# RenYurui/Global-Flow-Local-Attention

Hardware: AMD Instinct MI355X
Metric: images/sec (fwd+bwd) PoseGenerator 256x176 attn_layer=2,3 -- feature-warping hot path (higher is better)
Workload: dtype f32 (FC products: 2-term f16 splits exact to 2^-24 on f16 MFMA, f32 accumulate)

## Files before the change

### global_flow_local_attention_amd/csrc/fc_conv_impl.h

```cpp
#pragma once

#include "fc_mma.h"

namespace gfla {

constexpr int kFcMinRowBlocks = 2, kFcMaxRowBlocks = 8;
constexpr int kFcPrefetch = 8;

template <int MODE>
__device__ __forceinline__ void load_b_frags(Frag<MODE> (&fb)[Fc<MODE>::KB], const unsigned char *p, int64_t split_stride) {
  if constexpr (MODE == 0) {
    fb[0].v = *reinterpret_cast<const float4 *>(p);
    fb[1].v = *reinterpret_cast<const float4 *>(p + 32);
  } else {
#pragma unroll
    for (int sp = 0; sp < Fc<MODE>::NS; ++sp) fb[0].s[sp] = *reinterpret_cast<const f16x8 *>(p + sp * split_stride);
  }
}

typedef unsigned int u32x4 __attribute__((ext_vector_type(4)));

__device__ __forceinline__ void fc_prefetch_pieces(u32x4 (&pf)[kFcPrefetch], const unsigned char *src, int x_ps, int pix0,
                                                   int tmh) {
#pragma unroll
  for (int q = 0; q < kFcPrefetch; ++q)
    pf[q] = *reinterpret_cast<const u32x4 *>(src + (int64_t)min(pix0 + 64 * q, tmh - 1) * x_ps);
}

struct ConvTiling {
  int T, base, rem, heavy, per_ntile;
};

template <int MODE, int KS, int NMB, bool SRC32 = false>
__global__ __launch_bounds__(256, 2) void fc_conv_kernel(PackedDesc X, const unsigned char *__restrict__ Wk,
                                                        int64_t w_split_stride, float *__restrict__ out,
                                                        int64_t out_bs, int ldo, int n_valid, int M, int Wv, int Wp,
                                                        int nch, int tmh, ConvTiling tl,
                                                        const uint32_t *__restrict__ amax_x,
                                                        const uint32_t *__restrict__ amax_w) {
  using F = Fc<MODE>;
  constexpr int KK = KS * KS, PITCH = F::PITCH, STEPS = F::KB * NMB;
  extern __shared__ __attribute__((aligned(16))) unsigned char gfla_smem[];
  unsigned char *xs = gfla_smem;
  const int t = threadIdx.x, lane = t & 63, wave = t >> 6, l31 = lane & 31, kh = lane >> 5;
  int wid = blockIdx.x;
  const int ntile = wid / tl.per_ntile;
  wid -= ntile * tl.per_ntile;
  if (tl.per_ntile <= 2 * kNumCU && wid >= kNumCU) wid = tl.per_ntile - 1 - (wid - kNumCU);
  else if (tl.per_ntile <= kNumCU && (ntile & 1)) wid = tl.per_ntile - 1 - wid;
  int64_t b;
  int first, nblk;
  if (wid < tl.heavy) {
    b = wid / tl.rem;
    first = (wid - (int)b * tl.rem) * (tl.base + 1);
    nblk = tl.base + 1;
  } else {
    const int u = wid - tl.heavy, per = tl.T - tl.rem;
    b = u / per;
    first = tl.rem * (tl.base + 1) + (u - (int)b * per) * tl.base;
    nblk = tl.base;
  }
  const int m0 = first * 32;
  const int y0 = m0 / Wv, p0 = y0 * Wp + (m0 - y0 * Wv);
  const int64_t x_ss = X.split_stride, x_cs = X.chunk_stride;
  const int x_ps = X.pix_stride;
  const unsigned char *xg = X.base + b * X.batch_stride + (int64_t)p0 * x_ps;
  constexpr int64_t kWTile = (int64_t)kFcTN * F::REC;
  const unsigned char *wg = Wk + (int64_t)ntile * nch * KK * kWTile + (wave * 32 + l31) * F::REC + kh * 16;

  int a_off[NMB];
#pragma unroll
  for (int mb = 0; mb < NMB; ++mb) {
    const int r = min(m0 + mb * 32 + l31, M - 1);
    const int y = r / Wv;
    a_off[mb] = (y * Wp + (r - y * Wv) - p0) * PITCH;
  }

  f32x16 acc[NMB];
#pragma unroll
  for (int mb = 0; mb < NMB; ++mb)
#pragma unroll
    for (int r = 0; r < 16; ++r) acc[mb][r] = 0.f;

  static_assert(!SRC32 || MODE == 2, "float32 source: mode 2 arithmetic only");
  const int per = tmh * (SRC32 ? 4 : F::PIECES);
  const int x_total = SRC32 ? per : per * F::NS;
  const int xplane = tmh * PITCH;

  constexpr int PF = kFcPrefetch;
  constexpr bool kPrefetch = MODE == 0 || SRC32;
  const float sx32 = SRC32 ? fc_scale(amax_x) : 1.f;
  auto store_split = [&](unsigned char *dst8, u32x4 v) {
    uint32_t h01, l01, h23, l23;
    fc_split_pair(__uint_as_float(v[0]) * sx32, __uint_as_float(v[1]) * sx32, h01, l01);
    fc_split_pair(__uint_as_float(v[2]) * sx32, __uint_as_float(v[3]) * sx32, h23, l23);
    *reinterpret_cast<uint2 *>(dst8) = make_uint2(h01, h23);
    *reinterpret_cast<uint2 *>(dst8 + xplane) = make_uint2(l01, l23);
  };
  u32x4 pf[PF];
  const int pix0 = t >> 2;
  const unsigned char *pf_src = xg + (t & 3) * 16;
  unsigned char *pf_dst = xs + (size_t)pix0 * PITCH + (t & 3) * (SRC32 ? 8 : 16);
  const int x_first = kPrefetch ? min(x_total, 256 * PF) : 0;

  Frag<MODE> cur[F::KB], nxt[F::KB];
  load_b_frags<MODE>(cur, wg, w_split_stride);
  if constexpr (kPrefetch) fc_prefetch_pieces(pf, pf_src, x_ps, pix0, tmh);
  for (int cc = 0; cc < nch; ++cc) {
    __syncthreads();
    if constexpr (kPrefetch) {
#pragma unroll
      for (int q = 0; q < PF; ++q)
        if (pix0 + 64 * q < tmh) {
          if constexpr (SRC32) store_split(pf_dst + (size_t)q * 64 * PITCH, pf[q]);
          else *reinterpret_cast<u32x4 *>(pf_dst + (size_t)q * 64 * PITCH) = pf[q];
        }
    }
    if constexpr (SRC32) {
      const unsigned char *src = xg + (int64_t)cc * x_cs + (t & 3) * 16;
      for (int pix = pix0 + 64 * PF; pix < tmh; pix += 64)
        store_split(xs + (size_t)pix * PITCH + (t & 3) * 8, *reinterpret_cast<const u32x4 *>(src + (int64_t)pix * x_ps));
    } else if (x_first < x_total) {
      const unsigned char *src = xg + (int64_t)cc * x_cs;
      for (int base = x_first + t; base < x_total; base += 256 * 4) {
        uint4 v0 = make_uint4(0, 0, 0, 0), v1 = v0, v2 = v0, v3 = v0;
#define GFLA_X_SP(idx_) (((idx_) >= per) + ((idx_) >= 2 * per))
#define GFLA_X_REM(idx_) ((idx_)-GFLA_X_SP(idx_) * per)
#define GFLA_X_SRC(idx_) \
  (src + GFLA_X_SP(idx_) * x_ss + (int64_t)(GFLA_X_REM(idx_) / F::PIECES) * x_ps + (GFLA_X_REM(idx_) % F::PIECES) * 16)
#define GFLA_X_DST(idx_) \
  (xs + ((size_t)GFLA_X_SP(idx_) * tmh + GFLA_X_REM(idx_) / F::PIECES) * PITCH + (GFLA_X_REM(idx_) % F::PIECES) * 16)
        if (base < x_total) v0 = *reinterpret_cast<const uint4 *>(GFLA_X_SRC(base));
        if (base + 256 < x_total) v1 = *reinterpret_cast<const uint4 *>(GFLA_X_SRC(base + 256));
        if (base + 512 < x_total) v2 = *reinterpret_cast<const uint4 *>(GFLA_X_SRC(base + 512));
        if (base + 768 < x_total) v3 = *reinterpret_cast<const uint4 *>(GFLA_X_SRC(base + 768));
        if (base < x_total) *reinterpret_cast<uint4 *>(GFLA_X_DST(base)) = v0;
        if (base + 256 < x_total) *reinterpret_cast<uint4 *>(GFLA_X_DST(base + 256)) = v1;
        if (base + 512 < x_total) *reinterpret_cast<uint4 *>(GFLA_X_DST(base + 512)) = v2;
        if (base + 768 < x_total) *reinterpret_cast<uint4 *>(GFLA_X_DST(base + 768)) = v3;
#undef GFLA_X_SRC
#undef GFLA_X_DST
#undef GFLA_X_SP
#undef GFLA_X_REM
      }
    }
    __syncthreads();
    Frag<MODE> fa = load_frag<MODE>(xs + a_off[0], xplane, 0, kh);
#pragma unroll 1
    for (int tap = 0; tap < KK; ++tap) {
      {
        const int lin = cc * KK + tap + 1;
#pragma unroll
        for (int q = 0; q < F::KB; ++q) nxt[q] = cur[q];
        if (lin < nch * KK) load_b_frags<MODE>(nxt, wg + (int64_t)lin * kWTile, w_split_stride);
        if constexpr (kPrefetch)
          if (tap == 0 && cc + 1 < nch)
            fc_prefetch_pieces(pf, pf_src + (int64_t)(cc + 1) * x_cs, x_ps, pix0, tmh);
      }
      const int i = tap / KS, j = tap - i * KS;
      const unsigned char *xa = xs + (size_t)(i * Wp + j) * PITCH;
      const int tn = tap + 1 < KK ? tap + 1 : 0;
      const int in = tn / KS, jn = tn - in * KS;
      const unsigned char *xa_next = xs + (size_t)(in * Wp + jn) * PITCH;
#pragma unroll
      for (int st = 0; st < STEPS; ++st) {
        const int kb = st / NMB, mb = st % NMB;
        const Frag<MODE> fc = fa;
        if (st + 1 < STEPS)
          fa = load_frag<MODE>(xa + a_off[(st + 1) % NMB], xplane, (st + 1) / NMB, kh);
        else
          fa = load_frag<MODE>(xa_next + a_off[0], xplane, 0, kh);
        __builtin_amdgcn_sched_barrier(0);
        if (mb + 1 < NMB || nblk == NMB)
          acc[mb] = mma<MODE>(fc, cur[kb], acc[mb]);
      }
#pragma unroll
      for (int q = 0; q < F::KB; ++q) cur[q] = nxt[q];
    }
  }

  const float inv = MODE == 0 ? 1.f : fc_inv_scale(amax_x) * fc_inv_scale(amax_w);
  float *ob = out + b * out_bs;
  const int col = ntile * kFcTN + wave * 32 + l31;
  if (col < n_valid) {
#pragma unroll
    for (int mb = 0; mb < NMB; ++mb) {
      if (mb >= nblk) continue;
#pragma unroll
      for (int r = 0; r < 16; ++r) {
        const int m = m0 + mb * 32 + (r & 3) + 8 * (r >> 2) + 4 * kh;
        if (m < M) ob[(int64_t)m * ldo + col] = acc[mb][r] * inv;
      }
    }
  }
}



inline int fc_conv_tile_pixels(int mb, int Wv, int Wp, int k) {
  const int tm = 32 * mb;
  return tm + ((tm - 1) / Wv + 1) * (Wp - Wv) + (k - 1) * (Wp + 1);
}

inline int pick_conv_tiling(int M, int64_t B, int ntiles_n, int Wv, int Wp, int k, int mode, ConvTiling *tl) {
  const int ns = fc_nsplit(mode), pitch = mode ? 48 : 80;
  const int nb = (int)ceil_div(M, 32);
  const int forced = tuning(11);
  int64_t T = (2 * kNumCU) / (B * ntiles_n);
  if (T < 1) T = 1;
  if (T > nb) T = nb;
  if (ceil_div(nb, T) > kFcMaxRowBlocks) T = ceil_div(nb, kFcMaxRowBlocks);
  if (forced >= kFcMinRowBlocks && forced <= kFcMaxRowBlocks) T = ceil_div(nb, forced);
  for (;; ++T) {
    const int nmb = (int)ceil_div(nb, T);
    const int64_t lds = (int64_t)ns * fc_conv_tile_pixels(nmb < kFcMinRowBlocks ? kFcMinRowBlocks : nmb, Wv, Wp, k) * pitch;
    if (lds <= 156 * 1024) break;
    if (nmb <= kFcMinRowBlocks) return 0;
  }
  tl->T = (int)T;
  tl->base = nb / (int)T;
  tl->rem = nb % (int)T;
  tl->heavy = (int)B * tl->rem;
  tl->per_ntile = (int)(B * T);
  int nmb = tl->base + (tl->rem ? 1 : 0);
  if (nmb < kFcMinRowBlocks) {
    nmb = kFcMinRowBlocks;
  }
  return nmb;
}

template <int MODE, int KS, int NMB, bool SRC32 = false>
static int launch_conv(const PackedDesc &X, const void *wk, int64_t w_split_stride, float *out, int64_t out_bs,
                       int ldo, int n_valid, int64_t B, int nch, int M, int Wv, int Wp, const ConvTiling &tl,
                       const uint32_t *amax_x, const uint32_t *amax_w, hipStream_t stream) {
  using F = Fc<MODE>;
  const int tmh = fc_conv_tile_pixels(NMB, Wv, Wp, KS);
  const unsigned lds = (unsigned)(F::NS * tmh * F::PITCH);
  const int64_t wgs = (int64_t)tl.per_ntile * ceil_div(n_valid, kFcTN);
  if (wgs > 0x7fffffffLL) return GFLA_ERR_UNSUPPORTED;
  auto kern = fc_conv_kernel<MODE, KS, NMB, SRC32>;
  if (lds > 64 * 1024)
    (void)hipFuncSetAttribute(reinterpret_cast<const void *>(kern), hipFuncAttributeMaxDynamicSharedMemorySize, (int)lds);
  kern<<<dim3((unsigned)wgs), 256, lds, stream>>>(X, static_cast<const unsigned char *>(wk), w_split_stride, out, out_bs,
                                                  ldo, n_valid, M, Wv, Wp, nch, tmh, tl, amax_x, amax_w);
  return launch_status();
}

template <int MODE, int KS, bool SRC32 = false>
static int dispatch_conv(int nmb, const PackedDesc &X, const void *wk, int64_t wss, float *out, int64_t out_bs, int ldo,
                         int n_valid, int64_t B, int nch, int M, int Wv, int Wp, const ConvTiling &tl, const uint32_t *ax,
                         const uint32_t *aw, hipStream_t s) {
  switch (nmb) {
#define GFLA_CASE(N_) \
  case N_: return launch_conv<MODE, KS, N_, SRC32>(X, wk, wss, out, out_bs, ldo, n_valid, B, nch, M, Wv, Wp, tl, ax, aw, s)
    GFLA_CASE(2);
    GFLA_CASE(3);
    GFLA_CASE(4);
    GFLA_CASE(5);
    GFLA_CASE(6);
    GFLA_CASE(7);
    GFLA_CASE(8);
#undef GFLA_CASE
  }
  return GFLA_ERR_UNSUPPORTED;
}

template <int MODE>
int fc_conv_mode(const PackedDesc &X, const void *wk, int64_t w_split_stride, float *out, int64_t out_bs, int ldo,
                 int n_valid, int64_t B, int nch, int M, int Wv, int Wp, int k, const uint32_t *amax_x,
                 const uint32_t *amax_w, hipStream_t stream);

#define GFLA_DEFINE_FC_CONV_MODE(MODE_)                                                                               \
  template <>                                                                                                         \
  int fc_conv_mode<MODE_>(const PackedDesc &X, const void *wk, int64_t w_split_stride, float *out, int64_t out_bs,    \
                          int ldo, int n_valid, int64_t B, int nch, int M, int Wv, int Wp, int k,                     \
                          const uint32_t *amax_x, const uint32_t *amax_w, hipStream_t stream) {                       \
    ConvTiling tl;                                                                                                    \
    const int nmb = pick_conv_tiling(M, B, (int)ceil_div(n_valid, kFcTN), Wv, Wp, k, MODE_, &tl);                      \
    if (nmb == 0) return GFLA_ERR_UNSUPPORTED;                                                                        \
    if (k == 3)                                                                                                       \
      return dispatch_conv<MODE_, 3>(nmb, X, wk, w_split_stride, out, out_bs, ldo, n_valid, B, nch, M, Wv, Wp, tl,     \
                                     amax_x, amax_w, stream);                                                         \
    return dispatch_conv<MODE_, 5>(nmb, X, wk, w_split_stride, out, out_bs, ldo, n_valid, B, nch, M, Wv, Wp, tl,       \
                                   amax_x, amax_w, stream);                                                           \
  }

}
```

Measured before the change: 9591.

## Ring-buffer weight fragments two taps ahead and load via buffer resources

```diff
diff --git a/global_flow_local_attention_amd/csrc/fc_conv_impl.h b/global_flow_local_attention_amd/csrc/fc_conv_impl.h
--- a/global_flow_local_attention_amd/csrc/fc_conv_impl.h
+++ b/global_flow_local_attention_amd/csrc/fc_conv_impl.h
@@ -6,25 +6,33 @@
 
 constexpr int kFcMinRowBlocks = 2, kFcMaxRowBlocks = 8;
 constexpr int kFcPrefetch = 8;
+constexpr int kFcWeightAhead = 2, kFcRingMaxRowBlocks = 7;
+
+typedef unsigned int u32x4 __attribute__((ext_vector_type(4)));
+
+__device__ __forceinline__ __amdgpu_buffer_rsrc_t fc_rsrc(const unsigned char *base) {
+  return __builtin_amdgcn_make_buffer_rsrc(const_cast<unsigned char *>(base), 0, -1, 0x00020000);
+}
 
 template <int MODE>
-__device__ __forceinline__ void load_b_frags(Frag<MODE> (&fb)[Fc<MODE>::KB], const unsigned char *p, int64_t split_stride) {
+__device__ __forceinline__ void load_b_frags(Frag<MODE> (&fb)[Fc<MODE>::KB], const __amdgpu_buffer_rsrc_t (&w)[Fc<MODE>::NS],
+                                             int tile_off, int lane_off) {
   if constexpr (MODE == 0) {
-    fb[0].v = *reinterpret_cast<const float4 *>(p);
-    fb[1].v = *reinterpret_cast<const float4 *>(p + 32);
+    fb[0].v = __builtin_bit_cast(float4, __builtin_amdgcn_raw_buffer_load_b128(w[0], lane_off, tile_off, 0));
+    fb[1].v = __builtin_bit_cast(float4, __builtin_amdgcn_raw_buffer_load_b128(w[0], lane_off + 32, tile_off, 0));
   } else {
 #pragma unroll
-    for (int sp = 0; sp < Fc<MODE>::NS; ++sp) fb[0].s[sp] = *reinterpret_cast<const f16x8 *>(p + sp * split_stride);
-  }
-}
-
-typedef unsigned int u32x4 __attribute__((ext_vector_type(4)));
-
-__device__ __forceinline__ void fc_prefetch_pieces(u32x4 (&pf)[kFcPrefetch], const unsigned char *src, int x_ps, int pix0,
-                                                   int tmh) {
+    for (int sp = 0; sp < Fc<MODE>::NS; ++sp)
+      fb[0].s[sp] = __builtin_bit_cast(f16x8, __builtin_amdgcn_raw_buffer_load_b128(w[sp], lane_off, tile_off, 0));
+  }
+}
+
+__device__ __forceinline__ void fc_prefetch_pieces(u32x4 (&pf)[kFcPrefetch], const unsigned char *tile, int x_ps, int pix0,
+                                                   int tmh, int piece_off) {
+  const __amdgpu_buffer_rsrc_t x = fc_rsrc(tile);
 #pragma unroll
   for (int q = 0; q < kFcPrefetch; ++q)
-    pf[q] = *reinterpret_cast<const u32x4 *>(src + (int64_t)min(pix0 + 64 * q, tmh - 1) * x_ps);
+    pf[q] = __builtin_amdgcn_raw_buffer_load_b128(x, min(pix0 + 64 * q, tmh - 1) * x_ps + piece_off, 0, 0);
 }
 
 struct ConvTiling {
@@ -66,7 +74,10 @@
   const int x_ps = X.pix_stride;
   const unsigned char *xg = X.base + b * X.batch_stride + (int64_t)p0 * x_ps;
   constexpr int64_t kWTile = (int64_t)kFcTN * F::REC;
-  const unsigned char *wg = Wk + (int64_t)ntile * nch * KK * kWTile + (wave * 32 + l31) * F::REC + kh * 16;
+  const int w_lane = (wave * 32 + l31) * F::REC + kh * 16;
+  __amdgpu_buffer_rsrc_t wg[F::NS];
+#pragma unroll
+  for (int sp = 0; sp < F::NS; ++sp) wg[sp] = fc_rsrc(Wk + (int64_t)ntile * nch * KK * kWTile + sp * w_split_stride);
 
   int a_off[NMB];
 #pragma unroll
@@ -99,13 +110,18 @@
   };
   u32x4 pf[PF];
   const int pix0 = t >> 2;
-  const unsigned char *pf_src = xg + (t & 3) * 16;
+  const int pf_piece = (t & 3) * 16;
   unsigned char *pf_dst = xs + (size_t)pix0 * PITCH + (t & 3) * (SRC32 ? 8 : 16);
   const int x_first = kPrefetch ? min(x_total, 256 * PF) : 0;
 
-  Frag<MODE> cur[F::KB], nxt[F::KB];
-  load_b_frags<MODE>(cur, wg, w_split_stride);
-  if constexpr (kPrefetch) fc_prefetch_pieces(pf, pf_src, x_ps, pix0, tmh);
+  constexpr int TU = KS == 3 && NMB <= kFcRingMaxRowBlocks ? KK : 1, AHEAD = TU == 1 ? 1 : kFcWeightAhead;
+  static_assert(KK % TU == 0 && AHEAD >= 1 && (TU == 1 || AHEAD < TU), "ring: a slot per tap phase, reused after it has been read");
+  const int lin_last = nch * KK - 1;
+  Frag<MODE> ring[TU + 1][F::KB];
+#pragma unroll
+  for (int q = 0; q < AHEAD; ++q)
+    load_b_frags<MODE>(ring[q], wg, min(q, lin_last) * (int)kWTile, w_lane);
+  if constexpr (kPrefetch) fc_prefetch_pieces(pf, xg, x_ps, pix0, tmh, pf_piece);
   for (int cc = 0; cc < nch; ++cc) {
     __syncthreads();
     if constexpr (kPrefetch) {
@@ -147,35 +163,45 @@
     __syncthreads();
     Frag<MODE> fa = load_frag<MODE>(xs + a_off[0], xplane, 0, kh);
 #pragma unroll 1
-    for (int tap = 0; tap < KK; ++tap) {
-      {
-        const int lin = cc * KK + tap + 1;
-#pragma unroll
-        for (int q = 0; q < F::KB; ++q) nxt[q] = cur[q];
-        if (lin < nch * KK) load_b_frags<MODE>(nxt, wg + (int64_t)lin * kWTile, w_split_stride);
-        if constexpr (kPrefetch)
-          if (tap == 0 && cc + 1 < nch)
-            fc_prefetch_pieces(pf, pf_src + (int64_t)(cc + 1) * x_cs, x_ps, pix0, tmh);
+    for (int t0 = 0; t0 < KK; t0 += TU) {
+#pragma unroll
+      for (int u = 0; u < TU; ++u) {
+        const int tap = t0 + u;
+        constexpr int kNextSlot = TU == 1 ? 1 : 0;
+        {
+          const int lin = min(cc * KK + tap + AHEAD, lin_last);
+          if constexpr (TU == 1) {
+#pragma unroll
+            for (int q = 0; q < F::KB; ++q) ring[1][q] = ring[0][q];
+          }
+          if (TU > 1 || cc * KK + tap + 1 <= lin_last)
+            load_b_frags<MODE>(ring[TU == 1 ? kNextSlot : (u + AHEAD) % TU], wg, lin * (int)kWTile, w_lane);
+          if constexpr (kPrefetch)
+            if (tap == 0 && cc + 1 < nch)
+              fc_prefetch_pieces(pf, xg + (int64_t)(cc + 1) * x_cs, x_ps, pix0, tmh, pf_piece);
+        }
+        const int i = tap / KS, j = tap - i * KS;
+        const unsigned char *xa = xs + (size_t)(i * Wp + j) * PITCH;
+        const int tn = tap + 1 < KK ? tap + 1 : 0;
+        const int in = tn / KS, jn = tn - in * KS;
+        const unsigned char *xa_next = xs + (size_t)(in * Wp + jn) * PITCH;
+#pragma unroll
+        for (int st = 0; st < STEPS; ++st) {
+          const int kb = st / NMB, mb = st % NMB;
+          const Frag<MODE> fc = fa;
+          if (st + 1 < STEPS)
+            fa = load_frag<MODE>(xa + a_off[(st + 1) % NMB], xplane, (st + 1) / NMB, kh);
+          else
+            fa = load_frag<MODE>(xa_next + a_off[0], xplane, 0, kh);
+          __builtin_amdgcn_sched_barrier(0);
+          if (mb + 1 < NMB || nblk == NMB)
+            acc[mb] = mma<MODE>(fc, ring[u][kb], acc[mb]);
+        }
+        if constexpr (TU == 1) {
+#pragma unroll
+          for (int q = 0; q < F::KB; ++q) ring[0][q] = ring[1][q];
+        }
       }
-      const int i = tap / KS, j = tap - i * KS;
-      const unsigned char *xa = xs + (size_t)(i * Wp + j) * PITCH;
-      const int tn = tap + 1 < KK ? tap + 1 : 0;
-      const int in = tn / KS, jn = tn - in * KS;
-      const unsigned char *xa_next = xs + (size_t)(in * Wp + jn) * PITCH;
-#pragma unroll
-      for (int st = 0; st < STEPS; ++st) {
-        const int kb = st / NMB, mb = st % NMB;
-        const Frag<MODE> fc = fa;
-        if (st + 1 < STEPS)
-          fa = load_frag<MODE>(xa + a_off[(st + 1) % NMB], xplane, (st + 1) / NMB, kh);
-        else
-          fa = load_frag<MODE>(xa_next + a_off[0], xplane, 0, kh);
-        __builtin_amdgcn_sched_barrier(0);
-        if (mb + 1 < NMB || nblk == NMB)
-          acc[mb] = mma<MODE>(fc, cur[kb], acc[mb]);
-      }
-#pragma unroll
-      for (int q = 0; q < F::KB; ++q) cur[q] = nxt[q];
     }
   }
 
```

Result: no change. 9568 (-0.2%).
